# gabrielspmoreira/chameleon_recsys

Measured on AMD Instinct MI355X. Metric: NAR training sessions/sec, higher is better.
Workload: dtype f32

## Files before the change

chameleon_recsys_amd/_lib.py:

```python
import ctypes
import os
from ctypes import c_double, c_float, c_int, c_int32, c_int64, c_long, c_size_t, c_uint32, c_void_p

_HERE = os.path.dirname(os.path.abspath(__file__))
LIB_PATH = os.path.join(_HERE, "libchameleon_nar.so")

P = c_void_p

_SIGNATURES = {
    "cham_neg_sample_workspace_bytes": (c_size_t, [c_int, c_int, c_int]),
    "cham_neg_sample": (c_int, [P, c_int, c_int, P, c_int, c_uint32, c_uint32, c_int, c_int, c_int, c_int, P, P, P, P, P,
                                P, c_size_t, P]),
    "cham_ctx_assemble": (c_int, [P, P, c_int, P, c_int, P, P, P, P, P, P]),
    "cham_set_log_bases": (c_int, [c_float, c_float]),
    "cham_step_ints": (c_int, [P, P, P, P, c_int64, c_int, c_int, P, c_int, P, P, P, P, P, P]),
    "cham_item_dynamic_raw": (c_int, [P, P, c_int, P, P, P, P, P]),
    "cham_norm_stats_from_recent": (c_int, [P, c_int, c_int64, P, P, P, P, P]),
    "cham_norm_stats_from_buffer": (c_int, [P, c_int, c_int64, P, P, P, P, P]),
    "cham_norm_stats_from_rows": (c_int, [P, P, P, c_int, P, P]),
    "cham_row_weights": (c_int, [P, c_int, P, c_size_t, c_int, P, P, P, P]),
    "cham_item_assemble": (c_int, [P, c_int, c_int, c_int, P, c_int, P, c_int, P, P, P, P, c_int, P, P, P, P, P, P]),
    "cham_item_assemble_lds": (c_int, [P, c_int, c_int, c_int, P, c_int, P, c_int, P, P, P, P, c_int, P, c_int, P, c_int, P, P, P, P, P, P]),
    "cham_feature_bwd": (c_int, [P, P, c_int, c_int, P, P, P]),
    "cham_feature_bwd_workspace_bytes": (c_size_t, [c_int]),
# ... 17 lines not shown
    "cham_gemm_f32x3_launch_counts": (None, [P, c_int]),
    "cham_gemm_p3": (c_int, [P, c_int64, c_int, P, c_int64, c_int, c_int, P, c_int, c_int, c_int, c_int, P, c_int, P, c_int, c_int, c_int,
                             P, c_size_t, c_int, P]),
    "cham_gemm_b16_dma": (c_int, [P, c_int, P, c_int, c_int, P, c_int, c_int, c_int, c_int, P, c_int, P, c_int, c_int, c_int, P, c_size_t, c_int, P]),
    "cham_gemm_p3_launch_counts": (None, [P, c_int]),
    "cham_gemm_b16_dma_set_nt_wide": (c_int, [c_int]),
    "cham_split3": (c_int, [P, c_int, c_int, c_int, P, c_int64, c_int, P, c_int64, c_int, P]),
    "cham_combine_fwd_p3": (c_int, [P, P, c_int, c_int, c_int, c_int, P, P, c_int64, P]),
    "cham_mulpred_bwd_p3": (c_int, [P, P, P, c_int, c_int, c_int, P, P, c_int64, P, P]),
    "cham_dm_mulpred_p3": (c_int, [P, c_int, c_int, P, c_int64, P, P, c_int, c_int, c_int, P, c_int64, P, P, P]),
    "cham_h2_scale_absmax": (c_int, [P, c_size_t, P, c_size_t, P, P]),
    "cham_h2_scale_rownorm": (c_int, [P, c_long, c_int, c_int, P, P, P]),
    "cham_h2_scale_rownorm2": (c_int, [P, c_long, c_int, c_int, P, P, P, P]),
    "cham_split2h": (c_int, [P, c_int, c_int, c_int, P, c_int64, c_int, P, c_int64, c_int, P, c_int, P]),
    "cham_gemm_h2": (c_int, [P, c_int64, c_int, P, P, c_int64, c_int, P, c_int, P, c_int, c_int, c_int, c_int, P, c_int, P, c_int, c_int, c_int,
                             P, c_size_t, c_int, P]),
    "cham_h2b_block_elements": (c_int, []),
    "cham_gemm_h2b": (c_int, [P, c_int64, c_int, P, P, c_int64, c_int, P, c_int, P, c_int, c_int, c_int, c_int, P, c_int, P, c_int, c_int, c_int,
                              P, c_size_t, c_int, c_int, c_int, c_int, P]),
    "cham_combine_fwd_h2b": (c_int, [P, P, c_int, c_int, c_int, c_int, P, P, c_int64, P, c_int, P]),
    "cham_dm_mulpred_h2_blk": (c_int, [P, c_int, c_int, P, c_int64, P, P, P, P, c_int, c_int, c_int, P, c_int64, P, P, P, P]),
    "cham_gemm_h2_launch_counts": (None, [P, c_int]),
    "cham_gemm_h2_set_nt_wide": (c_int, [c_int]),
    "cham_combine_fwd_h2": (c_int, [P, P, c_int, c_int, c_int, c_int, P, P, c_int64, P, P]),
    "cham_mulpred_bwd_h2": (c_int, [P, P, P, c_int, c_int, c_int, P, P, c_int64, P, P, P]),
    "cham_dm_mulpred_h2": (c_int, [P, c_int, c_int, P, c_int64, P, P, c_int, c_int, c_int, P, c_int64, P, P, P, P]),
    "cham_dm_mulpred_h2h": (c_int, [P, c_int, c_int, P, c_int64, P, P, P, P, c_int, c_int, c_int, P, c_int64, P, P, P, P]),
    "cham_dm_mulpred_b16": (c_int, [P, c_int, c_int, P, P, P, c_int, c_int, c_int, P, P, P, P]),
    "cham_gemm_b16": (c_int, [P, c_int, c_int, P, c_int, c_int, P, c_int, c_int, c_int, c_int, c_int, P, c_int, P, c_int, c_int, c_int,
                              P, c_size_t, c_int, P]),
    "cham_gemm_b16_set_variant": (None, [c_int]),
    "cham_gemm_b16_launch_counts": (None, [P, c_int]),
    "cham_gemm_set_variant": (None, [c_int]),
    "cham_gemm_launch_counts": (None, [P, c_int]),
    "cham_combine_fwd": (c_int, [P, P, c_int, c_int, c_int, c_int, P, P, c_long, c_long, P]),
    "cham_combine_bwd_workspace_bytes": (c_size_t, [c_int, c_int, c_int, c_int]),
    "cham_combine_bwd": (c_int, [P, c_int, c_int, c_int, c_int, P, P, P, P, c_size_t, P]),
    "cham_combine_bwd_gs": (c_int, [P, c_int, c_int, c_int, c_int, P, P, P, P, c_size_t, P, c_size_t, P]),
    "cham_gemm_h2_groupsum_bytes": (c_size_t, [c_int, c_int, c_int]),
    "cham_gemm_h2_dgrad_gs": (c_int, [P, c_int64, c_int, P, P, c_int64, c_int, P, P, c_int, c_int, c_int, c_int, P, c_int, c_int, c_int, c_int, P,
                                      c_size_t, P]),
    "cham_combine_fwd_b16": (c_int, [P, P, c_int, c_int, c_int, c_int, P, P, P]),
    "cham_combine_bwd_b16": (c_int, [P, P, c_int, c_int, c_int, c_int, P, P, P, P, c_size_t, P]),
    "cham_mulpred_bwd_b16": (c_int, [P, P, P, c_int, c_int, c_int, P, P]),
    "cham_mul_rows_b16": (c_int, [P, P, c_int, c_int, c_int, P, P]),
    "cham_score_softmax_fwd_b16": (c_int, [P, c_int, P, P, c_int, c_int, c_float, P, P, P, P, c_float, P, P, P, P]),
# ... 65 lines not shown


class ChameleonLibError(RuntimeError):
    pass


_lib = None


def load():
    global _lib
    if _lib is not None:
        return _lib
    if not os.path.exists(LIB_PATH):
        raise ChameleonLibError(
            "HIP extension %s is missing - run `python -c 'import __graft_entry__ as g; g.build()'` "
            "(hipcc --offload-arch=gfx950).  There is no CPU fallback." % LIB_PATH)
    lib = ctypes.CDLL(LIB_PATH)
    for name, (res, args) in _SIGNATURES.items():
        fn = getattr(lib, name)
        fn.restype = res
        fn.argtypes = args
    lib.cham_gemm_h2_set_nt_wide(1 if os.environ.get("CHAM_H2_NT_WIDE", "1") == "1" else 0)
    lib.cham_gemm_b16_dma_set_nt_wide(1 if os.environ.get("CHAM_B16_NT_WIDE", "1") == "1" else 0)
    _lib = lib
    return lib


def check(rc, what):
    if rc != 0:
        raise ChameleonLibError("%s failed with code %d" % (what, rc))


def ptr(t):
    return None if t is None else t.data_ptr()
```

chameleon_recsys_amd/csrc/gemm_dma.h:

```cpp
#pragma once
#include "gemm_shared.h"
#include "gemm_dma_plan.h"

__device__ __forceinline__ u32x4 dma_rsrc(const void* base, unsigned bytes) {
    const unsigned long long a = (unsigned long long)base;
    u32x4 r;
    r.x = (unsigned)a; r.y = (unsigned)(a >> 32) & 0xFFFFu; r.z = bytes; r.w = 0x00020000u;
    return r;
}

__device__ __forceinline__ void dma_barrier() {
    __builtin_amdgcn_fence(__ATOMIC_RELEASE, "workgroup", "local");
    __builtin_amdgcn_s_waitcnt(0xc07f);
    __builtin_amdgcn_s_barrier();
    __builtin_amdgcn_fence(__ATOMIC_ACQUIRE, "workgroup", "local");
    __builtin_amdgcn_sched_barrier(0);
}

template <class V8, bool TN>
__device__ __forceinline__ V8 dma_frag(const unsigned char* __restrict__ s, unsigned hi_off = 4 * 512) {
    if constexpr (!TN) {
        return *reinterpret_cast<const V8*>(s);
    } else {
        typedef __attribute__((address_space(3))) s16x4 lds_s4;
// ... 15 lines not shown
        "s_mov_b32 m0, %1\n\ts_nop 0\n\tbuffer_load_dwordx4 %5, %7, 0 offen lds\n\t"
        "s_mov_b32 m0, %2\n\ts_nop 0\n\tbuffer_load_dwordx4 %6, %7, 0 offen lds\n\t"
        "s_mov_b32 m0, %3\n\ts_nop 0\n\tbuffer_load_dwordx4 %5, %8, 0 offen lds\n\t"
        "s_mov_b32 m0, %4\n\ts_nop 0\n\tbuffer_load_dwordx4 %6, %8, 0 offen lds\n\t"
        "s_mov_b32 m0, %0"
        : "=&s"(keep)
        : "s"(l0), "s"(l0b), "s"(l1), "s"(l1b), "v"(v0), "v"(v1), "s"(r0), "s"(r1)
        : "memory");
}
template <class P>
__device__ __forceinline__ GemmParams epilogue_params(const P& p, const float* bias) {
    GemmParams g;
    g.A = nullptr; g.B = nullptr; g.C = p.C; g.M = p.M; g.N = p.N; g.K = p.K; g.lda = 0; g.ldb = 0; g.ldc = p.ldc;
    g.bias = bias; g.act = ACT_NONE; g.dref = nullptr; g.ldr = 0; g.dact = ACT_NONE; g.rs = nullptr; g.ldrs = 0; g.rs_div = 1;
    g.accumulate = p.accumulate; g.kchunk = p.kchunk; g.splits = p.splits; g.partial = p.partial; g.nbm = p.nbm; g.nbn = p.nbn; g.xcd_split = p.xcd_split;
    g.sa = nullptr; g.sb = nullptr;
    return g;
}

static_assert(dma_plan::kOk == CHAM_OK && dma_plan::kErrArg == CHAM_ERR_ARG && dma_plan::kWindowBytes == WINDOW_BYTES, "gemm_dma_plan.h constants");
static_assert(dma_plan::kActNone == ACT_NONE && dma_plan::kActLeaky == ACT_LEAKY && dma_plan::kActTanh == ACT_TANH, "gemm_dma_plan.h constants");

template <auto KERNEL, int SMEM, int EPI, class P>
static int dma_launch(const P& p, int grid_y, long long (&counts)[8], hipStream_t st) {
    counts[6] = EPI; counts[7] = grid_y;
    CHAM_SET_DYNAMIC_LDS(KERNEL, SMEM);
    hipLaunchKernelGGL(KERNEL, dim3(p.nbm * p.nbn, grid_y, 1), dim3(512), SMEM, st, p);
    CHAM_CHECK_LAUNCH();
    return CHAM_OK;
}

static inline void launch_splitk_reduce(float* C, int ldc, int M, int N, int K, int accumulate, const dma_plan::SplitPlan& plan, float* workspace,
                                        int nbm, int nbn, hipStream_t st) {
    GemmParams g = {};
    g.C = C; g.M = M; g.N = N; g.K = K; g.ldc = ldc; g.act = ACT_NONE; g.dact = ACT_NONE; g.rs_div = 1; g.accumulate = accumulate;
    g.kchunk = plan.kchunk; g.splits = plan.splits; g.partial = workspace; g.nbm = nbm; g.nbn = nbn; g.xcd_split = plan.xcd_split;
    launch_splitk_reduce(g, st);
}

template <auto K_PARTIAL, auto K_PLAIN, int SMEM, class P>
static int dma_launch_tn(P& p, const dma_plan::SplitPlan& plan, int accumulate, long long (&counts)[8], hipStream_t st) {
    p.kchunk = plan.kchunk; p.splits = plan.splits;
    if (plan.splits > 1) {
        p.xcd_split = plan.xcd_split;
        const int rc = dma_launch<K_PARTIAL, SMEM, 6>(p, plan.splits, counts, st);
        if (rc != CHAM_OK) return rc;
        launch_splitk_reduce(p.C, p.ldc, p.M, p.N, p.K, accumulate, plan, p.partial, p.nbm, p.nbn, st);
        CHAM_CHECK_LAUNCH();
        return CHAM_OK;
    }
// ... 4 lines not shown
```

chameleon_recsys_amd/csrc/gemm_h2.hip:

```cpp
#include "gemm_dma.h"

typedef _Float16 half8 __attribute__((ext_vector_type(8)));

struct H2Params {
    const _Float16* A; const _Float16* B;
    long long a_ps, b_ps;
    int lda, ldb;
    const float* sa; const float* sb;
    float* C; int ldc;
    int M, N, K;
    const float* bias;
    const unsigned short* dref; int ldr;
    int kchunk, splits; float* partial;
    int nbm, nbn, xcd_split, accumulate;
    int a_tiles, b_tiles, r_blk;
    float* gsum; int ggrp, gsk;
};

#define H2_SLAB 8192
#define H2_STAGE (4 * H2_SLAB)
#define H2_RING 4

__device__ __forceinline__ void h2_dma_stage(unsigned lds0, unsigned va, unsigned vb, const u32x4& ra0, const u32x4& ra1, const u32x4& rb0,
                                             const u32x4& rb1) {
    unsigned keep;
    const unsigned l1 = lds0 + H2_SLAB, l2 = lds0 + 2 * H2_SLAB, l3 = lds0 + 3 * H2_SLAB;
    asm volatile(
        "s_nop 4\n\t"
        "s_mov_b32 %0, m0\n\t"
        "s_mov_b32 m0, %1\n\ts_nop 0\n\tbuffer_load_dwordx4 %5, %7, 0 offen lds\n\t"
        "s_mov_b32 m0, %2\n\ts_nop 0\n\tbuffer_load_dwordx4 %5, %8, 0 offen lds\n\t"
        "s_mov_b32 m0, %3\n\ts_nop 0\n\tbuffer_load_dwordx4 %6, %9, 0 offen lds\n\t"
        "s_mov_b32 m0, %4\n\ts_nop 0\n\tbuffer_load_dwordx4 %6, %10, 0 offen lds\n\t"
        "s_mov_b32 m0, %0"
        : "=&s"(keep)
        : "s"(lds0), "s"(l1), "s"(l2), "s"(l3), "v"(va), "v"(vb), "s"(ra0), "s"(ra1), "s"(rb0), "s"(rb1)
        : "memory");
}

template <int EPI, int TM, int TNN>
__device__ __forceinline__ void h2_epilogue(const H2Params& p, floatx16 (&acc)[TM][TNN], int m0, int n0, int wm0, int wn0, int split, int lane) {
    int lane_e = lane;
    asm volatile("" : "+v"(lane_e));
    const int kl = lane_e >> 5, fl = lane_e & 31;
    const float ia = p.sa[1], ib = p.sb[1];
#pragma unroll
    for (int i = 0; i < TM; ++i)
#pragma unroll
        for (int j = 0; j < TNN; ++j)
#pragma unroll
            for (int e = 0; e < 16; ++e) acc[i][j][e] = (acc[i][j][e] * ia) * ib;
    if constexpr (EPI == 3) {
        const int limM = p.M - m0, limN = p.N - n0;
        const __amdgpu_buffer_rsrc_t cw = make_window(p.C + (size_t)m0 * p.ldc + n0);
        const bool rb = p.r_blk != 0;
        const __amdgpu_buffer_rsrc_t dw = make_window(rb ? p.dref + ((size_t)(m0 >> 8) * (size_t)(p.ldr >> 5) + (size_t)(n0 >> 5)) * H2B_BLOCK
                                                         : p.dref + (size_t)m0 * p.ldr + n0);
        const int rstride = rb ? 64 : p.ldr * 2;
        const bool gs = p.gsum != nullptr;
        const int G = gs ? p.ggrp : 1, rbase = m0 + wm0;
        float* gw = gs ? p.gsum + (size_t)(rbase >> 7) * (size_t)p.gsk * (size_t)p.N + n0 + wn0 + fl : nullptr;
        float cur[TNN], hik[TNN];
#pragma unroll
        for (int j = 0; j < TNN; ++j) { cur[j] = 0.f; hik[j] = 0.f; }
// ... 81 lines not shown
                unsigned short y[16];
                unsigned offs[16];
#pragma unroll
                for (int e = 0; e < 16; ++e) {
                    const int row = wm0 + i * 32 + (e & 3) + 8 * (e >> 2) + 4 * kl;
                    const bool ok = cok && row < limM;
                    offs[e] = ok ? ((unsigned)row * (unsigned)p.ldc + (unsigned)col) * 4u : OOB_OFF;
                    const unsigned ro = rb ? (unsigned)((wn0 >> 5) + j) * (unsigned)(H2B_BLOCK * 2) + (unsigned)row * 64u + (unsigned)fl * 2u
                                           : ((unsigned)row * (unsigned)p.ldr + (unsigned)col) * 2u;
                    y[e] = __builtin_amdgcn_raw_buffer_load_b16(dw, ok ? ro : OOB_OFF, 0, 0);
                }
                float v[16];
#pragma unroll
                for (int e = 0; e < 16; ++e) {
                    v[e] = acc[i][j][e] * ((short)y[e] > 0 ? 1.f : 0.2f);
                    __builtin_amdgcn_raw_buffer_store_b32(__float_as_uint(v[e]), cw, offs[e], 0, 0);
                }
                block_add(j, v);
            }
            block_end();
        }
        if (gs) emit();
    } else {
        gemm_epilogue<EPI, TM, TNN>(epilogue_params(p, p.bias), acc, m0, n0, wm0, wn0, split, kl, fl);
    }
}

template <bool TN, int EPI>
__global__ __launch_bounds__(512) void gemm_h2_kernel(H2Params p) {
    constexpr int BM = 256, BN = 256, BK = 16, TM = 4, TNN = 2;
    extern __shared__ __attribute__((aligned(1024))) unsigned char h2_smem[];

    int tile_m, tile_n, split;
    gemm_tile_map(p, tile_m, tile_n, split);
    const int m0 = tile_m * BM, n0 = tile_n * BN;
    const int kbeg = split * p.kchunk;
    const int kend = min(p.K, kbeg + p.kchunk);
    const int nk = (kend - kbeg + BK - 1) / BK;
    const int lane = threadIdx.x & 63, wave = __builtin_amdgcn_readfirstlane(threadIdx.x >> 6);
    const int wm0 = (wave >> 2) * 128, wn0 = (wave & 3) * 64;

    u32x4 ra[2], rb[2];
    unsigned va, vb, stepa, stepb;
    unsigned tba = 0, tbb = 0;
    int klim = 0;
    if constexpr (!TN) {
// ... 120 lines not shown
            for (int ii = 0; ii < TM; ++ii) AH[ii] = dma_frag<half8, TN>(Sc + 0 * H2_SLAB + fa[ii], hia);
#pragma unroll
            for (int j = 0; j < TNN; ++j) BL[j] = dma_frag<half8, TN>(Sc + 3 * H2_SLAB + fb[j], hib);
            mma(AL, BH);
            mma(AH, BH);
            asm volatile("s_waitcnt vmcnt(8)" ::: "memory");
            dma_barrier();
#pragma unroll
            for (int j = 0; j < TNN; ++j) BH[j] = dma_frag<half8, TN>(Sn + 2 * H2_SLAB + fb[j], hib);
#pragma unroll
            for (int ii = 0; ii < TM; ++ii) AL[ii] = dma_frag<half8, TN>(Sn + 1 * H2_SLAB + fa[ii], hia);
            mma(AH, BL);
            cur = nxt;
        }
        asm volatile("s_waitcnt vmcnt(0)" ::: "memory");
    }

    h2_epilogue<EPI, TM, TNN>(p, acc, m0, n0, wm0, wn0, split, lane);
}

#define H2W_SLAB 16384
#define H2W_BUF (4 * H2W_SLAB)

template <int EPI, bool ABLK>
__global__ __launch_bounds__(512) void gemm_h2w_kernel(H2Params p) {
    constexpr int BM = 256, BN = 256, TM = 4, TNN = 2;
    extern __shared__ __attribute__((aligned(1024))) unsigned char h2_smem[];

    int tile_m, tile_n, split;
    gemm_tile_map<false>(p, tile_m, tile_n, split);
    const int m0 = tile_m * BM, n0 = tile_n * BN;
    const int nd = p.K >> 5;
    const int lane = threadIdx.x & 63, wave = __builtin_amdgcn_readfirstlane(threadIdx.x >> 6);
    const int wm0 = (wave >> 2) * 128, wn0 = (wave & 3) * 64;

    u32x4 ra[2], rb[2];
    const size_t aall = (size_t)max(p.M - m0, 0) * p.lda * 2, ball = (size_t)max(p.N - n0, 0) * p.ldb * 2;
#pragma unroll
    for (int q = 0; q < 2; ++q) {
        if constexpr (ABLK) ra[q] = dma_rsrc(p.A + q * p.a_ps + (size_t)tile_m * (size_t)(p.lda >> 5) * H2B_BLOCK,
                                            (unsigned)min((size_t)(p.lda >> 5) * (H2B_BLOCK * 2), (size_t)0xFFFFFFF0u));
        else ra[q] = dma_rsrc(p.A + q * p.a_ps + (size_t)m0 * p.lda, (unsigned)min(aall, (size_t)0xFFFFFFF0u));
        rb[q] = dma_rsrc(p.B + q * p.b_ps + (size_t)n0 * p.ldb, (unsigned)min(ball, (size_t)0xFFFFFFF0u));
    }
    const unsigned row = 32u * (unsigned)wave + (unsigned)(lane >> 2), sp = (unsigned)((lane & 3) ^ ((lane >> 4) & 3));
    unsigned va0 = ABLK ? row * 64u + 16u * sp : (row * (unsigned)p.lda + 8u * sp) * 2u;
    unsigned va1 = va0 + (ABLK ? 16u * 64u : 16u * (unsigned)p.lda * 2u);
    constexpr unsigned stepA = ABLK ? (unsigned)(H2B_BLOCK * 2) : 64u;
    unsigned vb0 = (row * (unsigned)p.ldb + 8u * sp) * 2u, vb1 = vb0 + 16u * (unsigned)p.ldb * 2u;

    unsigned fa0[TM], fb0[TNN], fa1[TM], fb1[TNN];
    {
        const int l31 = lane & 31;
        const unsigned fo = (unsigned)l31 * 64u + (unsigned)((lane >> 5) ^ ((l31 >> 2) & 3)) * 16u;
#pragma unroll
        for (int i = 0; i < TM; ++i) { fa0[i] = (unsigned)(wm0 + 32 * i) * 64u + fo; fa1[i] = fa0[i] ^ 32u; }
#pragma unroll
        for (int j = 0; j < TNN; ++j) { fb0[j] = (unsigned)(wn0 + 32 * j) * 64u + fo; fb1[j] = fb0[j] ^ 32u; }
    }

    floatx16 acc[TM][TNN];
#pragma unroll
    for (int i = 0; i < TM; ++i)
#pragma unroll
        for (int j = 0; j < TNN; ++j)
#pragma unroll
            for (int e = 0; e < 16; ++e) acc[i][j][e] = 0.f;

    typedef __attribute__((address_space(3))) unsigned char lds_u8;
    const unsigned lds_base = (unsigned)(unsigned long long)(lds_u8*)h2_smem;
    const unsigned wave_off = (unsigned)wave * 2048u;
    half8 AH[TM], AL[TM], BH[TNN], BL[TNN];

    auto mma = [&](const half8 (&X)[TM], const half8 (&Y)[TNN]) {
#pragma unroll
        for (int ii = 0; ii < TM; ++ii)
#pragma unroll
            for (int j = 0; j < TNN; ++j) acc[ii][j] = __builtin_amdgcn_mfma_f32_32x32x16_f16(X[ii], Y[j], acc[ii][j], 0, 0, 0);
        __builtin_amdgcn_sched_barrier(0);
    };
    auto dma_a = [&](unsigned buf) {
        dma4(lds_base + buf + 0 * H2W_SLAB + wave_off, lds_base + buf + 1 * H2W_SLAB + wave_off, va0, va1, ra[0], ra[1]);
        va0 += stepA; va1 += stepA;
    };
    auto dma_b = [&](unsigned buf) {
        dma4(lds_base + buf + 2 * H2W_SLAB + wave_off, lds_base + buf + 3 * H2W_SLAB + wave_off, vb0, vb1, rb[0], rb[1]);
        vb0 += 64u; vb1 += 64u;
    };

    if (nd > 0) {
        dma_a(0u); dma_b(0u);
        if (nd > 1) {
            dma_a((unsigned)H2W_BUF);
            asm volatile("s_waitcnt vmcnt(4)" ::: "memory");
        } else {
            asm volatile("s_waitcnt vmcnt(0)" ::: "memory");
        }
        dma_barrier();
        {
#pragma unroll
            for (int j = 0; j < TNN; ++j) BH[j] = *reinterpret_cast<const half8*>(h2_smem + 2 * H2W_SLAB + fb0[j]);
#pragma unroll
            for (int i = 0; i < TM; ++i) AL[i] = *reinterpret_cast<const half8*>(h2_smem + 1 * H2W_SLAB + fa0[i]);
        }
        for (int j = 0; j < nd; ++j) {
            const unsigned b0 = (unsigned)(j & 1) * (unsigned)H2W_BUF, b1 = (unsigned)H2W_BUF - b0;
            const unsigned char* S0 = h2_smem + b0;
            const unsigned char* S1 = h2_smem + b1;
            __builtin_amdgcn_sched_barrier(0);
            if (j + 1 < nd) dma_b(b1);
            __builtin_amdgcn_sched_barrier(0);
#pragma unroll
            for (int ii = 0; ii < TM; ++ii) AH[ii] = *reinterpret_cast<const half8*>(S0 + 0 * H2W_SLAB + fa0[ii]);
#pragma unroll
            for (int jn = 0; jn < TNN; ++jn) BL[jn] = *reinterpret_cast<const half8*>(S0 + 3 * H2W_SLAB + fb0[jn]);
            mma(AL, BH);
            mma(AH, BH);
#pragma unroll
            for (int jn = 0; jn < TNN; ++jn) BH[jn] = *reinterpret_cast<const half8*>(S0 + 2 * H2W_SLAB + fb1[jn]);
#pragma unroll
            for (int ii = 0; ii < TM; ++ii) AL[ii] = *reinterpret_cast<const half8*>(S0 + 1 * H2W_SLAB + fa1[ii]);
            mma(AH, BL);
#pragma unroll
            for (int ii = 0; ii < TM; ++ii) AH[ii] = *reinterpret_cast<const half8*>(S0 + 0 * H2W_SLAB + fa1[ii]);
#pragma unroll
            for (int jn = 0; jn < TNN; ++jn) BL[jn] = *reinterpret_cast<const half8*>(S0 + 3 * H2W_SLAB + fb1[jn]);
            mma(AL, BH);
            mma(AH, BH);
            asm volatile("s_waitcnt vmcnt(0)" ::: "memory");
            dma_barrier();
            if (j + 2 < nd) dma_a(b0);
            __builtin_amdgcn_sched_barrier(0);
#pragma unroll
            for (int jn = 0; jn < TNN; ++jn) BH[jn] = *reinterpret_cast<const half8*>(S1 + 2 * H2W_SLAB + fb0[jn]);
#pragma unroll
            for (int ii = 0; ii < TM; ++ii) AL[ii] = *reinterpret_cast<const half8*>(S1 + 1 * H2W_SLAB + fa0[ii]);
            mma(AH, BL);
        }
        asm volatile("s_waitcnt vmcnt(0)" ::: "memory");
    }

    h2_epilogue<EPI, TM, TNN>(p, acc, m0, n0, wm0, wn0, 0, lane);
}

__device__ __forceinline__ void h2_finish_scale(H2Scale* rec, float bound) {
    float s = 1.f, inv = 1.f;
    if (bound > 0.f && bound < __builtin_inff()) {
        int e;
        (void)frexpf(bound, &e);
        int k = 15 - e;
        k = k < -110 ? -110 : (k > 110 ? 110 : k);
        s = ldexpf(1.f, k); inv = ldexpf(1.f, -k);
    }
    rec->scale = s; rec->inv = inv; rec->bound = bound;
}

__device__ __forceinline__ float h2_block_max(float v, float* red) {
    v = wave_max(v);
    const int lane = threadIdx.x & 63, w = threadIdx.x >> 6;
    if (lane == 0) red[w] = v;
    __syncthreads();
    float t = 0.f;
    for (int i = 0; i < (int)(blockDim.x >> 6); ++i) t = fmaxf(t, red[i]);
    __syncthreads();
    return t;
// ... 132 lines not shown
    if (recompute) {
        if (ld != Cc || (n & 3) || ((uintptr_t)X & 15)) return -CHAM_ERR_ARG;
        const int rc = cham_h2_scale_absmax(X, n, nullptr, 0, rec, stream);
        if (rc != CHAM_OK) return rc;
    }
    int blocks = (int)((n + 255) / 256);
    if (blocks > 8192) blocks = 8192;
    hipLaunchKernelGGL(k_split2h, dim3(blocks), dim3(256), 0, (hipStream_t)stream, X, R, Cc, ld, reinterpret_cast<_Float16*>(dst), plane_stride,
                       ldd, reinterpret_cast<_Float16*>(dstT), plane_strideT, lddT, reinterpret_cast<const H2Scale*>(rec));
    CHAM_CHECK_LAUNCH();
    return CHAM_OK;
}

extern "C" int cham_h2b_block_elements(void) { return H2B_BLOCK; }

static long long g_h2_launches[8];
extern "C" void cham_gemm_h2_launch_counts(long long* out8, int reset) {
    for (int i = 0; i < 8; ++i) { if (out8) out8[i] = g_h2_launches[i]; if (reset) g_h2_launches[i] = 0; }
}

static int g_h2_nt_wide = 1;
extern "C" int cham_gemm_h2_set_nt_wide(int on) { const int was = g_h2_nt_wide; g_h2_nt_wide = on ? 1 : 0; return was; }

constexpr int H2_SMEM = H2_RING * H2_STAGE, H2W_SMEM = 2 * H2W_BUF;
template <int EPI>
static int h2w_launch(const H2Params& p, hipStream_t st) {
    ++g_h2_launches[2];
    if (p.a_tiles > 0) { ++g_h2_launches[3]; return dma_launch<gemm_h2w_kernel<EPI, true>, H2W_SMEM, EPI>(p, 1, g_h2_launches, st); }
    return dma_launch<gemm_h2w_kernel<EPI, false>, H2W_SMEM, EPI>(p, 1, g_h2_launches, st);
}
template <int EPI>
static int h2_launch_nt(const H2Params& p, bool wide, hipStream_t st) {
    return wide ? h2w_launch<EPI>(p, st) : dma_launch<gemm_h2_kernel<false, EPI>, H2_SMEM, EPI>(p, 1, g_h2_launches, st);
}
extern "C" size_t cham_gemm_h2_groupsum_bytes(int M, int N, int group_rows) {
    if (M <= 0 || N <= 0 || group_rows < 32) return 0;
    return (size_t)2 * ((M + 255) / 256) * (size_t)(127 / group_rows + 2) * (size_t)N * sizeof(float);
}
static int h2_run(const void* A, long long a_plane_stride, int lda, const float* a_scale, const void* B, long long b_plane_stride,
                  int ldb, const float* b_scale, int tn, float* C, int ldc, int M, int N, int K, const float* bias, int act,
                  const void* dref_h, int ldr, int dact, int accumulate, float* workspace, size_t workspace_bytes, int splits_hint,
                  int a_tiles, int b_tiles, int dref_blocked, int group_rows, float* groupsum, size_t groupsum_bytes, void* stream) {
    const dma_plan::Args a = {A, B, C, a_plane_stride, b_plane_stride, lda, ldb, ldc, tn, M, N, K, bias, act, dref_h, ldr, dact, accumulate};
    if (dma_plan::check_args(a, 16, false) != CHAM_OK || !a_scale || !b_scale || a_tiles < 0 || b_tiles < 0) return -CHAM_ERR_ARG;
    if (groupsum && (tn || !dref_h || group_rows < 32 || groupsum_bytes < cham_gemm_h2_groupsum_bytes(M, N, group_rows) || ((uintptr_t)groupsum & 15)))
        return -CHAM_ERR_ARG;
    {
        const long a_rows = tn ? K : M, b_rows = tn ? K : N;
        if (a_tiles && ((lda & 31) || (long)a_tiles * 256 < a_rows || a_plane_stride < (long long)a_tiles * (lda >> 5) * H2B_BLOCK)) return -CHAM_ERR_ARG;
        if (b_tiles && ((ldb & 31) || (long)b_tiles * 256 < b_rows || b_plane_stride < (long long)b_tiles * (ldb >> 5) * H2B_BLOCK)) return -CHAM_ERR_ARG;
        if (!tn && (b_tiles || (a_tiles && (lda != K || (K & 31) || !g_h2_nt_wide)))) return -CHAM_ERR_ARG;
        if (dref_blocked && (!dref_h || (ldr & 31) || tn)) return -CHAM_ERR_ARG;
    }
    H2Params p;
    p.A = reinterpret_cast<const _Float16*>(A); p.B = reinterpret_cast<const _Float16*>(B); p.a_ps = a_plane_stride; p.b_ps = b_plane_stride;
    p.lda = lda; p.ldb = ldb; p.sa = a_scale; p.sb = b_scale; p.C = C; p.ldc = ldc; p.M = M; p.N = N; p.K = K; p.bias = bias;
    p.dref = reinterpret_cast<const unsigned short*>(dref_h); p.ldr = ldr; p.partial = workspace; p.xcd_split = 0; p.accumulate = 0;
    p.kchunk = K; p.splits = 1;
    p.nbm = (M + 255) / 256; p.nbn = (N + 255) / 256;
    p.a_tiles = a_tiles; p.b_tiles = b_tiles; p.r_blk = dref_blocked ? 1 : 0;
    p.gsum = groupsum; p.ggrp = group_rows; p.gsk = groupsum ? 127 / group_rows + 2 : 0;
    hipStream_t st = (hipStream_t)stream;
    if (!tn) {
        const int epi = dma_plan::nt_epilogue(bias != nullptr, act, dref_h != nullptr, dact, true);
        if (epi < 0) return -CHAM_ERR_ARG;
        ++g_h2_launches[0];
        if (groupsum) ++g_h2_launches[5];
        const bool wide = g_h2_nt_wide && (K & 31) == 0;
        switch (epi) {
            case 3: return h2_launch_nt<3>(p, wide, st);
            case 2: return h2_launch_nt<2>(p, wide, st);
            case 5: return h2_launch_nt<5>(p, wide, st);
            default: return h2_launch_nt<0>(p, wide, st);
        }
    }
    dma_plan::SplitPlan plan;
    if (dma_plan::plan_tn_splits(M, N, K, lda, ldb, workspace != nullptr, workspace_bytes, splits_hint, 16, 512, plan) != CHAM_OK) return -CHAM_ERR_ARG;
    if ((a_tiles || b_tiles) && ((size_t)plan.kchunk + 512 + 64) * (size_t)(lda > ldb ? lda : ldb) * 2 >= 0xFFFFFFF0ull) return -CHAM_ERR_ARG;
    ++g_h2_launches[1];
    if (a_tiles || b_tiles) ++g_h2_launches[4];
    return dma_launch_tn<gemm_h2_kernel<true, 6>, gemm_h2_kernel<true, 0>, H2_SMEM>(p, plan, accumulate, g_h2_launches, st);
}

extern "C" int cham_gemm_h2b(const void* A, long long a_plane_stride, int lda, const float* a_scale, const void* B, long long b_plane_stride,
// ... 22 lines not shown
```

chameleon_recsys_amd/csrc/gemm_shared.h:

```cpp
#pragma once
#include "common.h"
#include "gemm_tile_plan.h"

typedef unsigned int u32x4 __attribute__((ext_vector_type(4)));
typedef unsigned int u32x2 __attribute__((ext_vector_type(2)));
typedef short s16x4 __attribute__((ext_vector_type(4)));
#define OOB_OFF 0x80000000u
#define WINDOW_BYTES 0x7FFFF000
static_assert(tile_plan::kOk == CHAM_OK && tile_plan::kErrArg == CHAM_ERR_ARG && tile_plan::kWindowBytes == WINDOW_BYTES, "gemm_tile_plan.h constants");
static_assert(tile_plan::kActNone == ACT_NONE && tile_plan::kActLeaky == ACT_LEAKY && tile_plan::kActTanh == ACT_TANH, "gemm_tile_plan.h constants");

__device__ __forceinline__ __amdgpu_buffer_rsrc_t make_window(const void* base) {
    return __builtin_amdgcn_make_buffer_rsrc(const_cast<void*>(base), 0, WINDOW_BYTES, 0x00020000);
}
__device__ __forceinline__ float4 as_f4(u32x4 v) {
    return make_float4(__uint_as_float(v.x), __uint_as_float(v.y), __uint_as_float(v.z), __uint_as_float(v.w));
}
__device__ __forceinline__ float bf_lo(unsigned u) { return __uint_as_float(u << 16); }
__device__ __forceinline__ float bf_hi(unsigned u) { return __uint_as_float(u & 0xFFFF0000u); }
__device__ __forceinline__ unsigned pack_bf2(float a, float b) {
    typedef __bf16 bf16x2 __attribute__((ext_vector_type(2)));
    bf16x2 v; v[0] = (__bf16)a; v[1] = (__bf16)b;
    return __builtin_bit_cast(unsigned, v);
}

template <bool SPLITK = true, class P>
__device__ __forceinline__ void gemm_tile_map(const P& p, int& tile_m, int& tile_n, int& split) {
    const int nwg = p.nbm * p.nbn;
    int tm, tn, sp;
    if (SPLITK && p.xcd_split) {
        const int lin = blockIdx.x + gridDim.x * blockIdx.y, slot = lin >> 3;
        sp = (lin & 7) + 8 * (slot / nwg);
        const int t = slot % nwg;
        tm = t / p.nbn; tn = t % p.nbn;
    } else {
        const int id = blockIdx.x;
        const int q = nwg / 8, rr = nwg % 8, xcd = id % 8;
        const int swz = (xcd < rr ? xcd * (q + 1) : rr * (q + 1) + (xcd - rr) * q) + id / 8;
        tm = swz / p.nbn; tn = swz % p.nbn;
        sp = SPLITK ? blockIdx.y : 0;
    }
    tile_m = tm; tile_n = tn; split = sp;
}

struct GemmParams {
    const float* A; const float* B; float* C;
    int M, N, K, lda, ldb, ldc;
    const float* bias; int act;
    const float* dref; int ldr; int dact;
    const float* rs; int ldrs; int rs_div;
    int accumulate;
    int kchunk; int splits; float* partial;
    int nbm, nbn;
    int xcd_split;
    const float* sa; const float* sb;
};


template <int ACT> __device__ __forceinline__ float act_fwd_c(float v) {
    if (ACT == ACT_LEAKY) return v > 0.f ? v : 0.2f * v;
    if (ACT == ACT_TANH) return cham_tanhf(v);
    return v;
}
template <int ACT> __device__ __forceinline__ float act_bwd_c(float y) {
    if (ACT == ACT_LEAKY) return y > 0.f ? 1.f : 0.2f;
// ... 300 lines not shown
```

include/chameleon_nar.h:

```cpp
#ifndef CHAMELEON_NAR_H
#define CHAMELEON_NAR_H
#include <stddef.h>
#include <stdint.h>
#ifdef __cplusplus
extern "C" {
#endif

#define CHAM_ACT_NONE 0
#define CHAM_ACT_LEAKY 1
#define CHAM_ACT_TANH 2

size_t cham_neg_sample_workspace_bytes(int n_aci, int buf_size, int n_from_buffer);
int cham_neg_sample(const int64_t* aci, int Bg, int T1, const int64_t* buffer, int buf_size, uint32_t seed, uint32_t step,
                    int row_begin, int row_count, int N, int n_from_buffer, int64_t* neg_ids, int32_t* neg_slot,
                    int64_t* pool, int32_t* canon, int32_t* meta, void* workspace, size_t workspace_bytes, void* stream);

int cham_ctx_assemble(const int64_t* cat, const float* num, int R, const int64_t* desc, int F, const float* params,
                      const float* gamma, const float* beta, float* xraw, float* xs, void* stream);
int cham_set_log_bases(float elapsed_days_smooth_log_base, float popularity_smooth_log_base);

int cham_step_ints(const int64_t* ic_rows, const int64_t* ln_rows, const int64_t* pool, const int64_t* ets_rows, int64_t max_ts, int BT, int pmax,
                   const int32_t* seq_len_in, int B, const uint8_t* mask_in, int64_t* ids_all, int64_t* ref_ts, int32_t* seq_len, uint8_t* mask,
                   void* stream);

// ... 55 lines not shown

int cham_gemm_p3(const void* A, long long a_plane_stride, int lda, const void* B, long long b_plane_stride, int ldb, int tn, float* C,
                 int ldc, int M, int N, int K, const float* bias, int act, const void* dref_h, int ldr, int dact, int accumulate,
                 float* workspace, size_t workspace_bytes, int splits_hint, void* stream);

int cham_gemm_b16_dma(const void* A, int lda, const void* B, int ldb, int tn, void* C, int ldc, int M, int N, int K, const float* bias,
                      int act, const void* dref, int ldr, int dact, int accumulate, float* workspace, size_t workspace_bytes,
                      int splits_hint, void* stream);
void cham_gemm_p3_launch_counts(long long* out8, int reset);
int cham_gemm_b16_dma_set_nt_wide(int on);
int cham_split3(const float* X, int R, int Cc, int ld, void* dst, long long plane_stride, int ldd, void* dstT, long long plane_strideT,
                int lddT, void* stream);

int cham_h2_scale_absmax(const float* x0, size_t n0, const float* x1, size_t n1, void* rec, void* stream);
int cham_h2_scale_rownorm(const float* X, long R, int K, int ld, const float* factor, void* rec, void* stream);
int cham_h2_scale_rownorm2(const float* X, long R, int K, int ld, const float* factor, void* rec, void* rec_plain, void* stream);
int cham_split2h(const float* X, int R, int Cc, int ld, void* dst, long long plane_stride, int ldd, void* dstT, long long plane_strideT,
                 int lddT, void* rec, int recompute, void* stream);
int cham_gemm_h2(const void* A, long long a_plane_stride, int lda, const float* a_scale, const void* B, long long b_plane_stride, int ldb,
                 const float* b_scale, int tn, float* C, int ldc, int M, int N, int K, const float* bias, int act, const void* dref_h, int ldr,
                 int dact, int accumulate, float* workspace, size_t workspace_bytes, int splits_hint, void* stream);
void cham_gemm_h2_launch_counts(long long* out8, int reset);
int cham_gemm_h2_set_nt_wide(int on);
int cham_h2b_block_elements(void);
int cham_gemm_h2b(const void* A, long long a_plane_stride, int lda, const float* a_scale, const void* B, long long b_plane_stride, int ldb,
                  const float* b_scale, int tn, float* C, int ldc, int M, int N, int K, const float* bias, int act, const void* dref_h, int ldr,
                  int dact, int accumulate, float* workspace, size_t workspace_bytes, int splits_hint, int a_tiles, int b_tiles,
                  int dref_blocked, void* stream);
int cham_combine_fwd_h2b(const float* U, const float* V, int C, int BT, int N, int pmax, const int32_t* neg_slot, void* Z1p,
                         long long plane_stride, const void* scale_rec, int blocked, void* stream);
int cham_dm_mulpred_h2_blk(const float* dS1, int lds1, int K, const void* Wp, long long w_plane_stride, const void* ds1_scale_rec,
                           const void* w_scale_rec, const float* Z2c, const float* pred, int C, int BT, int N, void* dZ2p,
                           long long out_plane_stride, const void* out_scale_rec, float* dpred_pre, float* col_part, void* stream);
int cham_combine_fwd_h2(const float* U, const float* V, int C, int BT, int N, int pmax, const int32_t* neg_slot, void* Z1p,
                        long long plane_stride, const void* scale_rec, void* stream);
int cham_mulpred_bwd_h2(const float* dM, const float* Z2c, const float* pred, int C, int BT, int N, float* dpred_pre, void* dZ2p,
                        long long plane_stride, float* col_part, const void* scale_rec, void* stream);
int cham_dm_mulpred_h2(const float* dS1, int lds1, int K, const void* Wp, long long w_plane_stride, const float* Z2c, const float* pred,
                       int C, int BT, int N, void* dZ2p, long long out_plane_stride, const void* out_scale_rec, float* dpred_pre,
                       float* col_part, void* stream);
int cham_dm_mulpred_h2h(const float* dS1, int lds1, int K, const void* Wh, long long w_plane_stride, const void* ds1_scale_rec,
                        const void* w_scale_rec, const float* Z2c, const float* pred, int C, int BT, int N, void* dZ2p,
                        long long out_plane_stride, const void* out_scale_rec, float* dpred_pre, float* col_part, void* stream);
int cham_dm_mulpred_b16(const void* dS1, int lds1, int K, const void* Ws1b, const void* Z2c, const float* pred, int C, int BT, int N, void* dZ2c,
                        float* dpred_pre, float* col_part, void* stream);

// ... 175 lines not shown
```

Before: 34280.

## Add optional persistent tile loop with next-tile prefetch to wide h2 NT GEMM

```diff
diff --git a/chameleon_recsys_amd/_lib.py b/chameleon_recsys_amd/_lib.py
--- a/chameleon_recsys_amd/_lib.py
+++ b/chameleon_recsys_amd/_lib.py
@@ -63,6 +63,7 @@
     "cham_dm_mulpred_h2_blk": (c_int, [P, c_int, c_int, P, c_int64, P, P, P, P, c_int, c_int, c_int, P, c_int64, P, P, P, P]),
     "cham_gemm_h2_launch_counts": (None, [P, c_int]),
     "cham_gemm_h2_set_nt_wide": (c_int, [c_int]),
+    "cham_gemm_h2_set_nt_persistent": (c_int, [c_int]),
     "cham_combine_fwd_h2": (c_int, [P, P, c_int, c_int, c_int, c_int, P, P, c_int64, P, P]),
     "cham_mulpred_bwd_h2": (c_int, [P, P, P, c_int, c_int, c_int, P, P, c_int64, P, P, P]),
     "cham_dm_mulpred_h2": (c_int, [P, c_int, c_int, P, c_int64, P, P, c_int, c_int, c_int, P, c_int64, P, P, P, P]),
@@ -174,6 +175,8 @@
         fn.restype = res
         fn.argtypes = args
     lib.cham_gemm_h2_set_nt_wide(1 if os.environ.get("CHAM_H2_NT_WIDE", "1") == "1" else 0)
+    n_wg = int(os.environ.get("CHAM_H2_NT_PERSISTENT", "0"))
+    lib.cham_gemm_h2_set_nt_persistent(-1 if n_wg == 1 or n_wg < 0 else n_wg)
     lib.cham_gemm_b16_dma_set_nt_wide(1 if os.environ.get("CHAM_B16_NT_WIDE", "1") == "1" else 0)
     _lib = lib
     return lib
diff --git a/chameleon_recsys_amd/csrc/gemm_dma.h b/chameleon_recsys_amd/csrc/gemm_dma.h
--- a/chameleon_recsys_amd/csrc/gemm_dma.h
+++ b/chameleon_recsys_amd/csrc/gemm_dma.h
@@ -61,10 +61,10 @@
 static_assert(dma_plan::kActNone == ACT_NONE && dma_plan::kActLeaky == ACT_LEAKY && dma_plan::kActTanh == ACT_TANH, "gemm_dma_plan.h constants");
 
 template <auto KERNEL, int SMEM, int EPI, class P>
-static int dma_launch(const P& p, int grid_y, long long (&counts)[8], hipStream_t st) {
+static int dma_launch(const P& p, int grid_y, long long (&counts)[8], hipStream_t st, int grid_x = 0) {
     counts[6] = EPI; counts[7] = grid_y;
     CHAM_SET_DYNAMIC_LDS(KERNEL, SMEM);
-    hipLaunchKernelGGL(KERNEL, dim3(p.nbm * p.nbn, grid_y, 1), dim3(512), SMEM, st, p);
+    hipLaunchKernelGGL(KERNEL, dim3(grid_x > 0 ? grid_x : p.nbm * p.nbn, grid_y, 1), dim3(512), SMEM, st, p);
     CHAM_CHECK_LAUNCH();
     return CHAM_OK;
 }
diff --git a/chameleon_recsys_amd/csrc/gemm_h2.hip b/chameleon_recsys_amd/csrc/gemm_h2.hip
--- a/chameleon_recsys_amd/csrc/gemm_h2.hip
+++ b/chameleon_recsys_amd/csrc/gemm_h2.hip
@@ -15,6 +15,7 @@
     int nbm, nbn, xcd_split, accumulate;
     int a_tiles, b_tiles, r_blk;
     float* gsum; int ggrp, gsk;
+    int nt_wg;
 };
 
 #define H2_SLAB 8192
@@ -39,7 +40,8 @@
 }
 
 template <int EPI, int TM, int TNN>
-__device__ __forceinline__ void h2_epilogue(const H2Params& p, floatx16 (&acc)[TM][TNN], int m0, int n0, int wm0, int wn0, int split, int lane) {
+__device__ __forceinline__ void h2_epilogue(const H2Params& p, floatx16 (&acc)[TM][TNN], int m0, int n0, int wm0, int wn0, int split, int lane,
+                                            const float* bpre = nullptr) {
     int lane_e = lane;
     asm volatile("" : "+v"(lane_e));
     const int kl = lane_e >> 5, fl = lane_e & 31;
@@ -167,6 +169,28 @@
         }
         if (gs) emit();
     } else {
+        if constexpr (EPI == 2 || EPI == 5) {
+            if (bpre && p.M - m0 >= wm0 + TM * 32 && p.N - n0 >= wn0 + TNN * 32) {
+                const __amdgpu_buffer_rsrc_t cw = make_window(p.C + (size_t)m0 * p.ldc + n0);
+#pragma unroll
+                for (int i = 0; i < TM; ++i)
+#pragma unroll
+                    for (int j = 0; j < TNN; ++j) {
+                        const unsigned col = (unsigned)(wn0 + j * 32 + fl), rowb = (unsigned)(wm0 + i * 32 + 4 * kl);
+                        const unsigned voff = (rowb * (unsigned)p.ldc + col) * 4u;
+                        const float bv = bpre[j];
+#pragma unroll
+                        for (int e = 0; e < 16; ++e) {
+                            const int ce = (e & 3) + 8 * (e >> 2);
+                            float v = acc[i][j][e];
+                            if (EPI == 2) v = act_fwd_c<ACT_TANH>(v + bv);
+                            else v = v + bv;
+                            __builtin_amdgcn_raw_buffer_store_b32(__float_as_uint(v), cw, voff, ce * p.ldc * 4, 0);
+                        }
+                    }
+                return;
+            }
+        }
         gemm_epilogue<EPI, TM, TNN>(epilogue_params(p, p.bias), acc, m0, n0, wm0, wn0, split, kl, fl);
     }
 }
@@ -333,32 +357,52 @@
 #define H2W_SLAB 16384
 #define H2W_BUF (4 * H2W_SLAB)
 
+template <unsigned O0, unsigned O1>
+__device__ __forceinline__ void h2w_dma4(unsigned l, unsigned v0, unsigned v1, const u32x4& r0, const u32x4& r1) {
+    unsigned keep;
+    asm volatile(
+        "s_nop 4\n\t"
+        "s_mov_b32 %0, m0\n\t"
+        "s_add_u32 m0, %1, %6\n\ts_nop 0\n\tbuffer_load_dwordx4 %2, %4, 0 offen lds\n\t"
+        "s_add_u32 m0, %1, %7\n\ts_nop 0\n\tbuffer_load_dwordx4 %3, %4, 0 offen lds\n\t"
+        "s_add_u32 m0, %1, %8\n\ts_nop 0\n\tbuffer_load_dwordx4 %2, %5, 0 offen lds\n\t"
+        "s_add_u32 m0, %1, %9\n\ts_nop 0\n\tbuffer_load_dwordx4 %3, %5, 0 offen lds\n\t"
+        "s_mov_b32 m0, %0"
+        : "=&s"(keep)
+        : "s"(l), "v"(v0), "v"(v1), "s"(r0), "s"(r1), "n"(O0), "n"(O0 + 1024u), "n"(O1), "n"(O1 + 1024u)
+        : "memory", "scc");
+}
+
 template <int EPI, bool ABLK>
 __global__ __launch_bounds__(512) void gemm_h2w_kernel(H2Params p) {
     constexpr int BM = 256, BN = 256, TM = 4, TNN = 2;
     extern __shared__ __attribute__((aligned(1024))) unsigned char h2_smem[];
 
-    int tile_m, tile_n, split;
-    gemm_tile_map<false>(p, tile_m, tile_n, split);
-    const int m0 = tile_m * BM, n0 = tile_n * BN;
     const int nd = p.K >> 5;
     const int lane = threadIdx.x & 63, wave = __builtin_amdgcn_readfirstlane(threadIdx.x >> 6);
     const int wm0 = (wave >> 2) * 128, wn0 = (wave & 3) * 64;
+    const int ntiles = p.nbm * p.nbn, tstride = p.nt_wg > 0 ? p.nt_wg : ntiles;
 
     u32x4 ra[2], rb[2];
-    const size_t aall = (size_t)max(p.M - m0, 0) * p.lda * 2, ball = (size_t)max(p.N - n0, 0) * p.ldb * 2;
-#pragma unroll
-    for (int q = 0; q < 2; ++q) {
-        if constexpr (ABLK) ra[q] = dma_rsrc(p.A + q * p.a_ps + (size_t)tile_m * (size_t)(p.lda >> 5) * H2B_BLOCK,
-                                            (unsigned)min((size_t)(p.lda >> 5) * (H2B_BLOCK * 2), (size_t)0xFFFFFFF0u));
-        else ra[q] = dma_rsrc(p.A + q * p.a_ps + (size_t)m0 * p.lda, (unsigned)min(aall, (size_t)0xFFFFFFF0u));
-        rb[q] = dma_rsrc(p.B + q * p.b_ps + (size_t)n0 * p.ldb, (unsigned)min(ball, (size_t)0xFFFFFFF0u));
-    }
-    const unsigned row = 32u * (unsigned)wave + (unsigned)(lane >> 2), sp = (unsigned)((lane & 3) ^ ((lane >> 4) & 3));
-    unsigned va0 = ABLK ? row * 64u + 16u * sp : (row * (unsigned)p.lda + 8u * sp) * 2u;
-    unsigned va1 = va0 + (ABLK ? 16u * 64u : 16u * (unsigned)p.lda * 2u);
+    unsigned va0, va1, vb0, vb1;
     constexpr unsigned stepA = ABLK ? (unsigned)(H2B_BLOCK * 2) : 64u;
-    unsigned vb0 = (row * (unsigned)p.ldb + 8u * sp) * 2u, vb1 = vb0 + 16u * (unsigned)p.ldb * 2u;
+    auto set_desc = [&](int tile_m, int tile_n) {
+        const int m0 = tile_m * BM, n0 = tile_n * BN;
+        const size_t aall = (size_t)max(p.M - m0, 0) * p.lda * 2, ball = (size_t)max(p.N - n0, 0) * p.ldb * 2;
+#pragma unroll
+        for (int q = 0; q < 2; ++q) {
+            if constexpr (ABLK) ra[q] = dma_rsrc(p.A + q * p.a_ps + (size_t)tile_m * (size_t)(p.lda >> 5) * H2B_BLOCK,
+                                                (unsigned)min((size_t)(p.lda >> 5) * (H2B_BLOCK * 2), (size_t)0xFFFFFFF0u));
+            else ra[q] = dma_rsrc(p.A + q * p.a_ps + (size_t)m0 * p.lda, (unsigned)min(aall, (size_t)0xFFFFFFF0u));
+            rb[q] = dma_rsrc(p.B + q * p.b_ps + (size_t)n0 * p.ldb, (unsigned)min(ball, (size_t)0xFFFFFFF0u));
+        }
+    };
+    auto set_offsets = [&]() {
+        const unsigned row = 32u * (unsigned)wave + (unsigned)(lane >> 2), sp = (unsigned)((lane & 3) ^ ((lane >> 4) & 3));
+        va0 = ABLK ? row * 64u + 16u * sp : (row * (unsigned)p.lda + 8u * sp) * 2u;
+        va1 = va0 + (ABLK ? 16u * 64u : 16u * (unsigned)p.lda * 2u);
+        vb0 = (row * (unsigned)p.ldb + 8u * sp) * 2u; vb1 = vb0 + 16u * (unsigned)p.ldb * 2u;
+    };
 
     unsigned fa0[TM], fb0[TNN], fa1[TM], fb1[TNN];
     {
@@ -371,16 +415,9 @@
     }
 
     floatx16 acc[TM][TNN];
-#pragma unroll
-    for (int i = 0; i < TM; ++i)
-#pragma unroll
-        for (int j = 0; j < TNN; ++j)
-#pragma unroll
-            for (int e = 0; e < 16; ++e) acc[i][j][e] = 0.f;
 
     typedef __attribute__((address_space(3))) unsigned char lds_u8;
-    const unsigned lds_base = (unsigned)(unsigned long long)(lds_u8*)h2_smem;
-    const unsigned wave_off = (unsigned)wave * 2048u;
+    const unsigned lds_wave = (unsigned)(unsigned long long)(lds_u8*)h2_smem + (unsigned)wave * 2048u;
     half8 AH[TM], AL[TM], BH[TNN], BL[TNN];
 
     auto mma = [&](const half8 (&X)[TM], const half8 (&Y)[TNN]) {
@@ -391,67 +428,123 @@
         __builtin_amdgcn_sched_barrier(0);
     };
     auto dma_a = [&](unsigned buf) {
-        dma4(lds_base + buf + 0 * H2W_SLAB + wave_off, lds_base + buf + 1 * H2W_SLAB + wave_off, va0, va1, ra[0], ra[1]);
+        h2w_dma4<0u, (unsigned)H2W_SLAB>(lds_wave + buf, va0, va1, ra[0], ra[1]);
         va0 += stepA; va1 += stepA;
     };
     auto dma_b = [&](unsigned buf) {
-        dma4(lds_base + buf + 2 * H2W_SLAB + wave_off, lds_base + buf + 3 * H2W_SLAB + wave_off, vb0, vb1, rb[0], rb[1]);
+        h2w_dma4<2u * H2W_SLAB, 3u * H2W_SLAB>(lds_wave + buf, vb0, vb1, rb[0], rb[1]);
         vb0 += 64u; vb1 += 64u;
     };
 
-    if (nd > 0) {
+    auto dma_first = [&]() {
         dma_a(0u); dma_b(0u);
-        if (nd > 1) {
-            dma_a((unsigned)H2W_BUF);
-            asm volatile("s_waitcnt vmcnt(4)" ::: "memory");
+        if (nd > 1) dma_a((unsigned)H2W_BUF);
+    };
+    constexpr bool BIAS = EPI == 2 || EPI == 5;
+    auto load_bias = [&](int n0, float (&bv)[TNN]) {
+        const __amdgpu_buffer_rsrc_t bw = make_window(p.bias + n0);
+#pragma unroll
+        for (int j = 0; j < TNN; ++j) {
+            const int col = wn0 + j * 32 + (lane & 31);
+            bv[j] = __uint_as_float(__builtin_amdgcn_raw_buffer_load_b32(bw, n0 + col < p.N ? (unsigned)col * 4u : OOB_OFF, 0, 0));
+        }
+    };
+
+    int t = blockIdx.x, tile_m, tile_n;
+    if (t >= ntiles) return;
+    gemm_tile_of(p, t, tile_m, tile_n);
+    set_desc(tile_m, tile_n); set_offsets();
+    if (nd > 0) dma_first();
+    bool first = true;
+    for (;;) {
+        const int m0 = tile_m * BM, n0 = tile_n * BN;
+#pragma unroll
+        for (int i = 0; i < TM; ++i)
+#pragma unroll
+            for (int j = 0; j < TNN; ++j)
+#pragma unroll
+                for (int e = 0; e < 16; ++e) acc[i][j][e] = 0.f;
+        float bv[TNN];
+#pragma unroll
+        for (int j = 0; j < TNN; ++j) bv[j] = 0.f;
+        if (nd > 0) {
+            if (first) {
+                if (nd > 1) asm volatile("s_waitcnt vmcnt(4)" ::: "memory");
+                else asm volatile("s_waitcnt vmcnt(0)" ::: "memory");
+            } else {
+                asm volatile("s_waitcnt vmcnt(63)" ::: "memory");
+            }
+            dma_barrier();
+            if constexpr (BIAS) load_bias(n0, bv);
+            {
+#pragma unroll
+                for (int j = 0; j < TNN; ++j) BH[j] = *reinterpret_cast<const half8*>(h2_smem + 2 * H2W_SLAB + fb0[j]);
+#pragma unroll
+                for (int i = 0; i < TM; ++i) AL[i] = *reinterpret_cast<const half8*>(h2_smem + 1 * H2W_SLAB + fa0[i]);
+            }
+            for (int j = 0; j < nd; ++j) {
+                const unsigned b0 = (unsigned)(j & 1) * (unsigned)H2W_BUF, b1 = (unsigned)H2W_BUF - b0;
+                const unsigned char* S0 = h2_smem + b0;
+                const unsigned char* S1 = h2_smem + b1;
+                __builtin_amdgcn_sched_barrier(0);
+                if (j + 1 < nd) dma_b(b1);
+                __builtin_amdgcn_sched_barrier(0);
+#pragma unroll
+                for (int ii = 0; ii < TM; ++ii) AH[ii] = *reinterpret_cast<const half8*>(S0 + 0 * H2W_SLAB + fa0[ii]);
+#pragma unroll
+                for (int jn = 0; jn < TNN; ++jn) BL[jn] = *reinterpret_cast<const half8*>(S0 + 3 * H2W_SLAB + fb0[jn]);
+                mma(AL, BH);
+                mma(AH, BH);
+#pragma unroll
+                for (int jn = 0; jn < TNN; ++jn) BH[jn] = *reinterpret_cast<const half8*>(S0 + 2 * H2W_SLAB + fb1[jn]);
+#pragma unroll
+                for (int ii = 0; ii < TM; ++ii) AL[ii] = *reinterpret_cast<const half8*>(S0 + 1 * H2W_SLAB + fa1[ii]);
+                mma(AH, BL);
+#pragma unroll
+                for (int ii = 0; ii < TM; ++ii) AH[ii] = *reinterpret_cast<const half8*>(S0 + 0 * H2W_SLAB + fa1[ii]);
+#pragma unroll
+                for (int jn = 0; jn < TNN; ++jn) BL[jn] = *reinterpret_cast<const half8*>(S0 + 3 * H2W_SLAB + fb1[jn]);
+                mma(AL, BH);
+                mma(AH, BH);
+                asm volatile("s_waitcnt vmcnt(0)" ::: "memory");
+                dma_barrier();
+                if (j + 2 < nd) dma_a(b0);
+                __builtin_amdgcn_sched_barrier(0);
+                if (j + 1 < nd) {
+#pragma unroll
+                    for (int jn = 0; jn < TNN; ++jn) BH[jn] = *reinterpret_cast<const half8*>(S1 + 2 * H2W_SLAB + fb0[jn]);
+#pragma unroll
+                    for (int ii = 0; ii < TM; ++ii) AL[ii] = *reinterpret_cast<const half8*>(S1 + 1 * H2W_SLAB + fa0[ii]);
+                }
+                mma(AH, BL);
+            }
         } else {
-            asm volatile("s_waitcnt vmcnt(0)" ::: "memory");
-        }
-        dma_barrier();
+            if constexpr (BIAS) load_bias(n0, bv);
+        }
+        if constexpr (BIAS) {
+#pragma unroll
+            for (int j = 0; j < TNN; ++j) asm volatile("" : "+v"(bv[j]));
+        }
+        const int t_next = t + tstride;
+        const bool more = t_next < ntiles;
+        int next_m = 0, next_n = 0;
+        if (more) {
+            gemm_tile_of(p, t_next, next_m, next_n);
+            set_desc(next_m, next_n); set_offsets();
+            if (nd > 0) dma_first();
+        }
         {
-#pragma unroll
-            for (int j = 0; j < TNN; ++j) BH[j] = *reinterpret_cast<const half8*>(h2_smem + 2 * H2W_SLAB + fb0[j]);
-#pragma unroll
-            for (int i = 0; i < TM; ++i) AL[i] = *reinterpret_cast<const half8*>(h2_smem + 1 * H2W_SLAB + fa0[i]);
-        }
-        for (int j = 0; j < nd; ++j) {
-            const unsigned b0 = (unsigned)(j & 1) * (unsigned)H2W_BUF, b1 = (unsigned)H2W_BUF - b0;
-            const unsigned char* S0 = h2_smem + b0;
-            const unsigned char* S1 = h2_smem + b1;
-            __builtin_amdgcn_sched_barrier(0);
-            if (j + 1 < nd) dma_b(b1);
-            __builtin_amdgcn_sched_barrier(0);
-#pragma unroll
-            for (int ii = 0; ii < TM; ++ii) AH[ii] = *reinterpret_cast<const half8*>(S0 + 0 * H2W_SLAB + fa0[ii]);
-#pragma unroll
-            for (int jn = 0; jn < TNN; ++jn) BL[jn] = *reinterpret_cast<const half8*>(S0 + 3 * H2W_SLAB + fb0[jn]);
-            mma(AL, BH);
-            mma(AH, BH);
-#pragma unroll
-            for (int jn = 0; jn < TNN; ++jn) BH[jn] = *reinterpret_cast<const half8*>(S0 + 2 * H2W_SLAB + fb1[jn]);
-#pragma unroll
-            for (int ii = 0; ii < TM; ++ii) AL[ii] = *reinterpret_cast<const half8*>(S0 + 1 * H2W_SLAB + fa1[ii]);
-            mma(AH, BL);
-#pragma unroll
-            for (int ii = 0; ii < TM; ++ii) AH[ii] = *reinterpret_cast<const half8*>(S0 + 0 * H2W_SLAB + fa1[ii]);
-#pragma unroll
-            for (int jn = 0; jn < TNN; ++jn) BL[jn] = *reinterpret_cast<const half8*>(S0 + 3 * H2W_SLAB + fb1[jn]);
-            mma(AL, BH);
-            mma(AH, BH);
-            asm volatile("s_waitcnt vmcnt(0)" ::: "memory");
-            dma_barrier();
-            if (j + 2 < nd) dma_a(b0);
-            __builtin_amdgcn_sched_barrier(0);
-#pragma unroll
-            for (int jn = 0; jn < TNN; ++jn) BH[jn] = *reinterpret_cast<const half8*>(S1 + 2 * H2W_SLAB + fb0[jn]);
-#pragma unroll
-            for (int ii = 0; ii < TM; ++ii) AL[ii] = *reinterpret_cast<const half8*>(S1 + 1 * H2W_SLAB + fa0[ii]);
-            mma(AH, BL);
-        }
-        asm volatile("s_waitcnt vmcnt(0)" ::: "memory");
-    }
-
-    h2_epilogue<EPI, TM, TNN>(p, acc, m0, n0, wm0, wn0, 0, lane);
+            H2Params pe = p;
+            int ewm0 = wm0, ewn0 = wn0;
+            asm volatile("" : "+s"(pe.ldc), "+s"(pe.ldr), "+s"(pe.M), "+s"(pe.N), "+s"(pe.ggrp), "+s"(pe.gsk), "+s"(pe.r_blk), "+s"(ewm0), "+s"(ewn0));
+            h2_epilogue<EPI, TM, TNN>(pe, acc, m0, n0, ewm0, ewn0, 0, lane, BIAS ? bv : nullptr);
+        }
+        if (!more) break;
+        asm volatile("" : "+s"(next_m), "+s"(next_n));
+        set_desc(next_m, next_n);
+        t = t_next; tile_m = next_m; tile_n = next_n; first = false;
+    }
+    asm volatile("s_waitcnt vmcnt(0)" ::: "memory");
 }
 
 __device__ __forceinline__ void h2_finish_scale(H2Scale* rec, float bound) {
@@ -630,12 +723,31 @@
 static int g_h2_nt_wide = 1;
 extern "C" int cham_gemm_h2_set_nt_wide(int on) { const int was = g_h2_nt_wide; g_h2_nt_wide = on ? 1 : 0; return was; }
 
+static int g_h2_nt_persistent = 0;
+extern "C" {
+int cham_gemm_h2_set_nt_persistent(int n_wg) { const int was = g_h2_nt_persistent; g_h2_nt_persistent = n_wg < 0 ? -1 : n_wg; return was; }
+}
+static int h2_device_cus() {
+    static int cus[64];
+    int dev = 0;
+    if (hipGetDevice(&dev) != hipSuccess || dev < 0 || dev >= 64) dev = 0;
+    if (cus[dev] == 0) {
+        int n = 0;
+        cus[dev] = (hipDeviceGetAttribute(&n, hipDeviceAttributeMultiprocessorCount, dev) == hipSuccess && n > 0) ? n : 256;
+    }
+    return cus[dev];
+}
+
 constexpr int H2_SMEM = H2_RING * H2_STAGE, H2W_SMEM = 2 * H2W_BUF;
 template <int EPI>
-static int h2w_launch(const H2Params& p, hipStream_t st) {
+static int h2w_launch(const H2Params& p0, hipStream_t st) {
+    H2Params p = p0;
+    const int tiles = p.nbm * p.nbn, want = g_h2_nt_persistent < 0 ? h2_device_cus() : g_h2_nt_persistent;
+    p.nt_wg = want > 0 ? (want < tiles ? want : tiles) : 0;
+    const int grid = p.nt_wg > 0 ? p.nt_wg : tiles;
     ++g_h2_launches[2];
-    if (p.a_tiles > 0) { ++g_h2_launches[3]; return dma_launch<gemm_h2w_kernel<EPI, true>, H2W_SMEM, EPI>(p, 1, g_h2_launches, st); }
-    return dma_launch<gemm_h2w_kernel<EPI, false>, H2W_SMEM, EPI>(p, 1, g_h2_launches, st);
+    if (p.a_tiles > 0) { ++g_h2_launches[3]; return dma_launch<gemm_h2w_kernel<EPI, true>, H2W_SMEM, EPI>(p, 1, g_h2_launches, st, grid); }
+    return dma_launch<gemm_h2w_kernel<EPI, false>, H2W_SMEM, EPI>(p, 1, g_h2_launches, st, grid);
 }
 template <int EPI>
 static int h2_launch_nt(const H2Params& p, bool wide, hipStream_t st) {
@@ -668,6 +780,7 @@
     p.nbm = (M + 255) / 256; p.nbn = (N + 255) / 256;
     p.a_tiles = a_tiles; p.b_tiles = b_tiles; p.r_blk = dref_blocked ? 1 : 0;
     p.gsum = groupsum; p.ggrp = group_rows; p.gsk = groupsum ? 127 / group_rows + 2 : 0;
+    p.nt_wg = 0;
     hipStream_t st = (hipStream_t)stream;
     if (!tn) {
         const int epi = dma_plan::nt_epilogue(bias != nullptr, act, dref_h != nullptr, dact, true);
diff --git a/chameleon_recsys_amd/csrc/gemm_shared.h b/chameleon_recsys_amd/csrc/gemm_shared.h
--- a/chameleon_recsys_amd/csrc/gemm_shared.h
+++ b/chameleon_recsys_amd/csrc/gemm_shared.h
@@ -41,6 +41,13 @@
         sp = SPLITK ? blockIdx.y : 0;
     }
     tile_m = tm; tile_n = tn; split = sp;
+}
+template <class P>
+__device__ __forceinline__ void gemm_tile_of(const P& p, int id, int& tile_m, int& tile_n) {
+    const int nwg = p.nbm * p.nbn;
+    const int q = nwg / 8, rr = nwg % 8, xcd = id % 8;
+    const int swz = (xcd < rr ? xcd * (q + 1) : rr * (q + 1) + (xcd - rr) * q) + id / 8;
+    tile_m = swz / p.nbn; tile_n = swz % p.nbn;
 }
 
 struct GemmParams {
diff --git a/include/chameleon_nar.h b/include/chameleon_nar.h
--- a/include/chameleon_nar.h
+++ b/include/chameleon_nar.h
@@ -101,6 +101,7 @@
                  int dact, int accumulate, float* workspace, size_t workspace_bytes, int splits_hint, void* stream);
 void cham_gemm_h2_launch_counts(long long* out8, int reset);
 int cham_gemm_h2_set_nt_wide(int on);
+int cham_gemm_h2_set_nt_persistent(int n_wg);
 int cham_h2b_block_elements(void);
 int cham_gemm_h2b(const void* A, long long a_plane_stride, int lda, const float* a_scale, const void* B, long long b_plane_stride, int ldb,
                   const float* b_scale, int tn, float* C, int ldc, int M, int N, int K, const float* bias, int act, const void* dref_h, int ldr,
```

Result: no change. 34320 (median of 2 runs) (+0.1%).
